# The-Learning-And-Vision-Atelier-LAVA/BUFFER

Measured on AMD Instinct MI355X. Metric: registration pairs/sec, higher is better.
Workload: dtype f32

## Files before the change

### buffer_amd/_lib.py

```python
import ctypes as C
import os

_HERE = os.path.dirname(os.path.abspath(__file__))
LIB_PATH = os.environ.get("BUF_LIB_PATH") or os.path.join(_HERE, "libbuffer_hip.so")

BUF_OK = 0


class BufferHipError(RuntimeError):
    pass


class buf_grid_t(C.Structure):
    _fields_ = [
        ("ws", C.c_void_p), ("ws_bytes", C.c_size_t),
        ("ns", C.c_int), ("nb", C.c_int),
        ("cells_per_elem", C.c_int64),
        ("radius", C.c_float),
        ("supports", C.c_void_p),
        ("desc", C.c_void_p), ("s_off", C.c_void_p), ("table", C.c_void_p),
        ("sorted", C.c_void_p), ("order", C.c_void_p), ("scan_tmp", C.c_void_p),
    ]


# ... 36 lines not shown
    "buf_vn_gather_block": (_i, [_vp, _vp, _vp, _vp, _i, _i, _i, _i, _i, _i, _f, _vp, _vp, _vp, _vp, _f, _vp, _vp]),
    "buf_vn_gather_pre_supported": (_i, [_i, _i, _i]),
    "buf_vn_gather_pre_ws_bytes": (_sz, [_i, _i]),
    "buf_vn_gather_block_pre": (_i, [_vp, _vp, _vp, _vp, _i, _i, _i, _i, _i, _f, _vp, _vp, _vp, _vp, _f, _vp, _vp, _sz, _vp]),
    "buf_vn_pointwise": (_i, [_vp, _vp, _i, _i, _i, _vp, _i, _i, _i, _vp, _vp, _vp, _vp, _f, _vp, _vp, _vp]),
    "buf_gather_max": (_i, [_vp, _vp, _i, _i, _i, _i, _vp, _vp]),
    "buf_vn_std": (_i, [_vp, _vp, _i, _i, _vp, _vp]),
    "buf_score_head_ws_bytes": (_sz, [_i, _i]),
    "buf_score_head": (_i, [_vp, _i, _vp, _i, _vp, _vp, _vp, _vp, _f, _vp, _vp, _vp, _vp, _f, _vp, _vp, _vp, _vp, _vp, _i, _vp, _vp, _i, _f,
                            _vp, _vp, _sz, _vp]),
    "buf_patch_voxelize_ws_bytes": (_sz, [_i]),
    "buf_patch_voxelize": (_i, [_vp, _vp, _i, _i, _f, _vp, _i, _i, _vp, _f, _i, _vp, _vp, _vp, _vp, _vp, _vp, _vp,
                                _vp, _vp, _sz, _vp]),
    "buf_cylindrical_net_wg": (_i, [_vp, _i, _vp, _vp, _vp, _vp, _vp, _vp, _vp]),
    "buf_cylindrical_net_wg_form": (_i, [_vp, _i, _vp, _vp, _vp, _vp, _vp, _i, _vp, _vp]),
    "buf_cylindrical_net_wg_supports": (_i, [_vp, _vp]),
    "buf_cylindrical_net_wg_flags": (_i, [_vp, _vp, _vp]),
    "buf_cylindrical_net_split_safe": (_i, [_vp, _i, _vp, _vp, _vp, _vp, _vp, _vp, _vp, _vp, _vp, _vp, _vp, _vp]),
    "buf_cylindrical_net_split_safe_form": (_i, [_vp, _i, _vp, _vp, _vp, _vp, _vp, _vp, _i, _vp, _vp, _vp, _vp, _vp, _vp]),
    "buf_cost_volume_net_split_safe": (_i, [_vp, _vp, _i, _vp, _vp, _i, _vp, _vp, _vp, _vp, _vp, _vp, _vp, _vp]),
    "buf_cylindrical_net_split": (_i, [_vp, _i, _vp, _vp, _vp, _vp, _vp, _vp, _vp, _vp]),
    "buf_cylindrical_net_split_head": (_i, [_vp, _i, _vp, _vp, _vp, _vp, _vp, _vp, _vp, _vp, _vp, _vp]),
    "buf_split_gemm_count": (C.c_longlong, [_i, _i, _i, _i]),
    "buf_split_tile_gemm": (_i, [_vp, _i, _i, _i, _i, _vp]),
    "buf_cost_volume_net_split": (_i, [_vp, _vp, _i, _vp, _vp, _vp, _vp, _vp]),
    "buf_cost_volume_net_split_gather": (_i, [_vp, _i, _vp, _vp, _i, _vp, _vp, _vp, _vp, _vp]),
    "buf_split_filter_count": (C.c_longlong, [_i, _i]),
    "buf_split_tile_filters": (_i, [_vp, _i, _i, _vp]),
    "buf_winograd_tile_weights": (_i, [_vp, _i, _i, _vp]),
    "buf_winograd_f24_tile_weights": (_i, [_vp, _i, _i, _vp]),
    "buf_winograd_group": (_i, [_i, _i]),
    "buf_cost_winograd_group": (_i, [_i]),
    "buf_winograd_tile_filters": (_i, [_vp, _i, _i, _i, _i, _vp]),
    "buf_voxel_downsample_ws_bytes": (_sz, [_i, _i64]),
    "buf_voxel_downsample": (_i, [_vp, _vp, _i, _i, C.c_double, _vp, _vp, _vp, _i64, _vp, _sz, _vp]),
# ... 62 lines not shown
```

### buffer_amd/csrc/buffer_hip.hip

```cpp
#include <stdlib.h>
#include "core.hip"
#include "radius.hip"
#include "icp.hip"
#include "pairstats.hip"
#include "posegraph.hip"
#include "metrics.hip"
#include "subsample.hip"
#include "pointops.hip"
#include "vn.hip"
#include "voxelize.hip"
#include "registration.hip"
#include "convnet.hip"
#include "convnet_h3.hip"
#include "costnet_h3.hip"
#include "preprocess.hip"
#include "convnet_wg.hip"
#include "convnet_w24.hip"
#include "convnet_w24k.hip"
#include "convnet_w24p.hip"
#include "costnet.hip"
#include "split_safe.hip"
#include "fpfh.hip"
#include "fgr.hip"
```

### buffer_amd/csrc/convnet_w24p.hip

```cpp
#include "common.h"

#define W24P_XCH_C 64
#define W24P_XCH_WIDE 36
#define W24P_XCH_OWN 12

#define W24P_MFMA(PRE, ACC, A, B) asm volatile(PRE "v_mfma_f32_16x16x4_f32 %0, %1, %2, %0" : "+a"(ACC) : "v"(A), "v"(B));

__device__ __forceinline__ void w24p_pass(unsigned P0, unsigned P1, float sgn, __amdgpu_buffer_rsrc_t rs, unsigned wp0, unsigned wp1, unsigned wp_next,
                                          unsigned lofs4, unsigned lofs2, int niter, wgf4 (&W4)[4][2], wgf2 (&W2)[4][2], wgf4 (&acc)[4][6])
{
    wgf2 D[6];
    float V[2][6];
    W24_LOAD(D, P0, P1, 0)
#define W24P_XFORM(BUF)                                                                                   \
    {                                                                                                     \
        float r_[6];                                                                                      \
        _Pragma("unroll") for (int b = 0; b < 6; b++)                                                     \
            r_[b] = __builtin_fmaf(sgn, D[3 + (b >> 1)][b & 1], D[b >> 1][b & 1]);                       \
        const float c_ = wg_sub(r_[4], r_[2]), e_ = wg_sub(r_[3], r_[1]);                                 \
        const float a_ = __builtin_fmaf(-4.f, r_[2], r_[4]), b_ = __builtin_fmaf(-4.f, r_[1], r_[3]);     \
        V[BUF][0] = __builtin_fmaf(4.f, r_[0], __builtin_fmaf(-4.f, r_[2], c_));                          \
        V[BUF][1] = wg_add(a_, b_); V[BUF][2] = wg_sub(a_, b_);                                           \
        V[BUF][3] = __builtin_fmaf(2.f, e_, c_); V[BUF][4] = __builtin_fmaf(-2.f, e_, c_);                \
        V[BUF][5] = __builtin_fmaf(-4.f, e_, wg_sub(r_[5], r_[3]));                                       \
    }
    W24P_XFORM(0)
    int it = 0;
#pragma unroll 1
    do {
        const bool more = it + 1 < niter;
        const unsigned wcur0 = wp0 + 4 * it * W24_WSTRIDE, wcur1 = wp1 + 4 * it * W24_WSTRIDE;
        const unsigned wn0 = more ? wcur0 + 4 * W24_WSTRIDE : wp_next;
        const unsigned wn1 = more ? wcur1 + 4 * W24_WSTRIDE : wp_next;
        const unsigned adv = more ? 4u * WG_KSTEP : 0u;
        __builtin_amdgcn_sched_barrier(0);
#pragma unroll
        for (int s = 0; s < 4; s++) {
            if (s < 3) W24_LOAD(D, P0, P1, (s + 1) * WG_KSTEP)
            else {
                P0 += adv; P1 += adv;
// ... 7 lines not shown
                    if (n == 0 && j == 0) W24P_MFMA("s_nop 1\n\t", acc[n][j], W24_U(n, s & 1, j), V[s & 1][j])
                    else W24P_MFMA("", acc[n][j], W24_U(n, s & 1, j), V[s & 1][j])
                }
            __builtin_amdgcn_sched_barrier(0);
            W24P_XFORM((s + 1) & 1)
#pragma unroll
            for (int n = 0; n < 4; n++) {
                const unsigned o = n < 2 ? (s < 2 ? wcur0 + (s + 2) * W24_WSTRIDE : wn0 + (s - 2) * W24_WSTRIDE)
                                         : (s < 2 ? wcur1 + (s + 2) * W24_WSTRIDE : wn1 + (s - 2) * W24_WSTRIDE);
                W4[n][s & 1] = wg_ldw(rs, o + (n & 1) * 256, lofs4);
                W2[n][s & 1] = w24_ldw2(rs, o + 512 + (n & 1) * 128, lofs2);
            }
            __builtin_amdgcn_sched_barrier(0);
        }
    } while (++it < niter);
#undef W24P_XFORM
    asm volatile("s_nop 15"
                 : "+a"(acc[0][0]), "+a"(acc[0][1]), "+a"(acc[0][2]), "+a"(acc[0][3]), "+a"(acc[0][4]), "+a"(acc[0][5]), "+a"(acc[1][0]), "+a"(acc[1][1]), "+a"(acc[1][2]), "+a"(acc[1][3]), "+a"(acc[1][4]), "+a"(acc[1][5]), "+a"(acc[2][0]), "+a"(acc[2][1]), "+a"(acc[2][2]), "+a"(acc[2][3]), "+a"(acc[2][4]), "+a"(acc[2][5]), "+a"(acc[3][0]), "+a"(acc[3][1]), "+a"(acc[3][2]), "+a"(acc[3][3]), "+a"(acc[3][4]), "+a"(acc[3][5]));
}

__device__ __forceinline__ void w24p_round_direct(unsigned row5, __amdgpu_buffer_rsrc_t rs, unsigned wp, unsigned lofs, int niter, unsigned pstride,
                                                  const float* __restrict__ bias_lane, const wgf4 (&W0)[2], wgf4& Y)
{
    constexpr int wstride = W24_WSTRIDE;
    wgf4 Wr[3][2];
#pragma unroll
    for (int k = 0; k < 2; k++) {
        Wr[0][k] = W0[k];
        Wr[1][k] = wg_ldw(rs, wp + pstride + k * wstride, lofs);
        Wr[2][k] = wg_ldw(rs, wp + 2 * pstride + k * wstride, lofs);
    }
    float X[2][6];
    unsigned pa = row5;
    WG_LOADD(X[0], pa, 0)
    WG_LOADD(X[1], pa, WG_KSTEP)
    wgf4 acc[3];
    float zero = 0.f;
    asm volatile("" : "+v"(zero));
    acc[0] = (wgf4){ zero, zero, zero, zero };
    acc[1] = (wgf4){ zero, zero, zero, zero };
    acc[2] = *reinterpret_cast<const wgf4*>(bias_lane);
    float G[6];
#define W24P_TAPS(SLOT)                                                                                   \
    {                                                                                                     \
        const wgf4 u0_ = Wr[0][SLOT], u1_ = Wr[1][SLOT], u2_ = Wr[2][SLOT];                               \
        const float d1_ = wg_sub(u1_[1], u2_[1]), d2_ = wg_sub(u1_[2], u2_[2]);                           \
        G[0] = u0_[0]; G[1] = wg_sub(u0_[1], u0_[2]); G[2] = u0_[3];                                      \
        G[3] = wg_sub(u1_[0], u2_[0]); G[4] = wg_sub(d1_, d2_); G[5] = wg_sub(u1_[3], u2_[3]);            \
    }
#define W24P_RELOAD(SLOT, OFS)                                                                            \
    _Pragma("unroll") for (int blk = 0; blk < 3; blk++) Wr[blk][SLOT] = wg_ldw(rs, (OFS) + blk * pstride, lofs);
    W24P_TAPS(0)
    W24P_RELOAD(0, wp + 2 * wstride)
#pragma unroll 1
    for (int it = 0; it < niter; it++) {
        const bool more = it + 1 < niter;
// ... 208 lines not shown
```

### buffer_amd/csrc/convnet_wg.hip

```cpp
#include "common.h"
#include <type_traits>

#define WG_CS 160
#define WG_ROW 22
#define WG_ZERO 154
#define WG_MAXC 128
#define WG_LAYERS 8
#define WG_THREADS 256
#define WG_BUF (WG_MAXC * WG_CS)
#define WG_KSTEP (16 * WG_CS)
#define WG_BLOCKS 16

typedef float wgf4 __attribute__((ext_vector_type(4)));
typedef float wgf2 __attribute__((ext_vector_type(2)));
typedef const __attribute__((address_space(3))) wgf2* wg_lds_f2;

struct CylWgParams {
    const float* wt[WG_LAYERS];
    const float* bias[WG_LAYERS];
    int cin[WG_LAYERS], cout[WG_LAYERS], relu[WG_LAYERS];
    const int* only_if;
#ifdef WG_STAMP
    long long* stamps;
#endif
// ... 581 lines not shown
                    const size_t idx = ((((((size_t)(n / ng) * nblk + i) * k4 + c / 4) * ng + n % ng) * 4 + c % 4) * 16 + o % 16);
                    out_host[idx * 4 + j] = (float)u;
                }
        }
    return BUF_OK;
}

extern "C" int buf_winograd_tile_weights(const float* w_host, int cout, int cin, float* out_host)
{
    BUF_REQUIRE(cout > 0 && cin > 0 && cout % 16 == 0 && cin % 4 == 0, BUF_EINVAL, "buf_winograd_tile_weights: widths %d -> %d", cin, cout);
    return buf_winograd_tile_filters(w_host, cout, cin, wg_group(cin, cout), WG_BLOCKS / 4, out_host);
}

extern "C" int buf_winograd_group(int cin, int cout) { return wg_group(cin, cout); }

static int wg_check_widths(const int* cin, const int* cout)
{
    for (int l = 0; l < WG_LAYERS; l++) {
        const int ci = cin[l], co = cout[l];
        BUF_REQUIRE(ci > 0 && ci % 16 == 0 && ci <= WG_MAXC && (co == 32 || co == 64 || co == 128), BUF_EINVAL,
                    "buf_cylindrical_net_wg: layer %d has unsupported widths %d -> %d", l, ci, co);
        BUF_REQUIRE(co != 128 || ci % 32 == 0, BUF_EINVAL,
                    "buf_cylindrical_net_wg: layer %d has unsupported widths %d -> %d (128 output channels need Cin %% 32 == 0)", l, ci, co);
        BUF_REQUIRE(co != 32 || (ci % 32 == 0 && ci <= 64), BUF_EINVAL,
                    "buf_cylindrical_net_wg: layer %d has unsupported widths %d -> %d (32 output channels need Cin = 32 or 64)", l, ci, co);
        BUF_REQUIRE(l == 0 || ci == cout[l - 1], BUF_EINVAL, "buf_cylindrical_net_wg: layer %d width mismatch", l);
        BUF_REQUIRE(l == 0 || cout[l - 1] != 32 || co == 32, BUF_EINVAL,
                    "buf_cylindrical_net_wg: layer %d has unsupported widths %d -> %d (only 32-output layers may follow a 32-output layer)", l, ci, co);
    }
    BUF_REQUIRE(cout[WG_LAYERS - 1] == 32, BUF_EINVAL, "buf_cylindrical_net_wg: the last layer must have 32 channels");
    return BUF_OK;
}

extern "C" int buf_cylindrical_net_wg_supports(const int* cin_host, const int* cout_host)
{
    BUF_REQUIRE(cin_host && cout_host, BUF_EINVAL, "buf_cylindrical_net_wg_supports: null argument");
    return wg_check_widths(cin_host, cout_host);
}

#define WG_F24_FLAG BUF_CYL_F24
static inline bool wg_f24_flagged(int relu) { return relu >= 2; }
static int w24_launch(const float* x, int npatch, CylWgParams P, float* y, void* stream, int form);
// ... 75 lines not shown
```

### buffer_amd/csrc/core.hip

```cpp
#include "common.h"
#include <stdarg.h>

static thread_local char g_err[512] = "";

void buf_set_error(const char* fmt, ...)
{
    va_list ap;
    va_start(ap, fmt);
    vsnprintf(g_err, sizeof(g_err), fmt, ap);
    va_end(ap);
}

extern "C" const char* buf_last_error(void) { return g_err; }
extern "C" int buf_version(void) { return 640; }

#include <mutex>
#include <vector>
struct TimedSpan { hipEvent_t a, b; double bytes; int id; };
static std::mutex g_time_mu;
static std::vector<TimedSpan> g_spans;
static int g_timing_on = 0;

extern "C" void buf_timing_enable(int on) { std::lock_guard<std::mutex> l(g_time_mu); g_timing_on = on; }

static bool timing_begin(hipStream_t s, TimedSpan* sp, double bytes, int id = BUF_TIMED_GRID_QUERY)
{
    if (!g_timing_on) return false;
    sp->id = id;
    if (hipEventCreate(&sp->a) != hipSuccess || hipEventCreate(&sp->b) != hipSuccess) return false;
// ... 241 lines not shown
```

### buffer_amd/csrc/split_safe.hip

```cpp
#include "common.h"

extern "C" int buf_cylindrical_net_split_safe_form(const float* x, int npatch, const void* const* wt_split_host, const float* const* wt_wg_host,
                                                   const float* const* bias_host, const int* cin_host, const int* cout_host, const int* relu_host,
                                                   int form, const float* head_params, float* y_or_equi, float* desc, int* status_dev,
                                                   int* flags_ws, void* stream)
{
    BUF_REQUIRE(npatch >= 0, BUF_EINVAL, "buf_cylindrical_net_split_safe: npatch=%d", npatch);
    if (npatch == 0) return BUF_OK;
    BUF_REQUIRE(x && y_or_equi && flags_ws && wt_split_host && wt_wg_host && bias_host && cin_host && cout_host && relu_host, BUF_EINVAL,
                "buf_cylindrical_net_split_safe: null argument");
    BUF_REQUIRE(!head_params || desc, BUF_EINVAL, "buf_cylindrical_net_split_safe: head without desc");
    BUF_REQUIRE(form >= BUF_CYL_FORM_DEFAULT && form <= BUF_CYL_FORM_PASS_SPLIT, BUF_EINVAL,
                "buf_cylindrical_net_split_safe: form=%d (-1: the library's default, 0: K split, 1: pass split)", form);
    if (int rc = buf_cylindrical_net_wg_flags(cin_host, cout_host, relu_host)) return rc;
    hipStream_t s = (hipStream_t)stream;
    BUF_CHECK_HIP(hipMemsetAsync(flags_ws, 0, sizeof(int) * (size_t)npatch, s));
    int relu_split[WG_LAYERS];
    for (int l = 0; l < WG_LAYERS; l++) relu_split[l] = wg_f24_flagged(relu_host[l]) ? (relu_host[l] & 1) : relu_host[l];
    int rc = h3_launch(x, npatch, wt_split_host, bias_host, cin_host, cout_host, relu_split, head_params ? nullptr : y_or_equi, head_params,
                       desc, head_params ? y_or_equi : nullptr, status_dev, stream, flags_ws);
    if (rc) return rc;
    rc = wg_launch(x, npatch, wt_wg_host, bias_host, cin_host, cout_host, relu_host, y_or_equi, flags_ws, stream, form);
    if (rc) return rc;
    if (head_params) {
        k_desc_head_masked<<<npatch, DH_THREADS, 0, s>>>(y_or_equi, head_params, desc, y_or_equi, flags_ws);
        BUF_LAUNCH_CHECK();
    }
    return BUF_OK;
}

extern "C" int buf_cylindrical_net_split_safe(const float* x, int npatch, const void* const* wt_split_host, const float* const* wt_wg_host,
                                              const float* const* bias_host, const int* cin_host, const int* cout_host, const int* relu_host,
                                              const float* head_params, float* y_or_equi, float* desc, int* status_dev, int* flags_ws,
                                              void* stream)
{
    return buf_cylindrical_net_split_safe_form(x, npatch, wt_split_host, wt_wg_host, bias_host, cin_host, cout_host, relu_host, BUF_CYL_FORM_DEFAULT,
                                               head_params, y_or_equi, desc, status_dev, flags_ws, stream);
}

extern "C" int buf_cost_volume_net_split_safe(const float* s_eq, const float* t_eq, int ele_n, const long long* s_rows, const long long* t_rows,
                                              int m, const void* const* wt_split_host, const float* const* bias_split_host,
                                              const float* const* wt_f32_host, const float* const* bias_f32_host, float* ind_out,
                                              int* status_dev, int* flags_ws, void* stream)
{
    BUF_REQUIRE(m >= 0, BUF_EINVAL, "buf_cost_volume_net_split_safe: m=%d", m);
    if (m == 0) return BUF_OK;
    BUF_REQUIRE(s_eq && t_eq && wt_split_host && bias_split_host && wt_f32_host && bias_f32_host && ind_out && flags_ws, BUF_EINVAL,
                "buf_cost_volume_net_split_safe: null argument");
    BUF_REQUIRE((s_rows == nullptr) == (t_rows == nullptr), BUF_EINVAL, "buf_cost_volume_net_split_safe: one row list without the other");
    BUF_REQUIRE(!s_rows || ele_n == 7, BUF_EINVAL, "buf_cost_volume_net_split_safe: ele_n=%d (the kernels are built for ele_n = 7)", ele_n);
    hipStream_t s = (hipStream_t)stream;
    BUF_CHECK_HIP(hipMemsetAsync(flags_ws, 0, sizeof(int) * (size_t)m, s));
    int rc = cost_net_h3_launch(s_eq, t_eq, m, wt_split_host, bias_split_host, s_rows, t_rows, ele_n, ind_out, status_dev, stream,
                                "buf_cost_volume_net_split_safe", flags_ws);
// ... 4 lines not shown
```

### buffer_amd/ops.py

```python
import ctypes as C
import time
import os
import numpy as np
import torch

from . import _lib
from ._lib import buf_grid_t, check


def _stream():
    return C.c_void_p(torch.cuda.current_stream().cuda_stream)


def _dev(t, dtype, what):
    if not isinstance(t, torch.Tensor) or not t.is_cuda:
        raise _lib.BufferHipError(f"{what}: expected a tensor in device memory (buffer_amd has no CPU path)")
    if t.dtype != dtype:
        t = t.to(dtype)
    return t.contiguous()


def _ptr(t):
    return C.c_void_p(t.data_ptr()) if t is not None else C.c_void_p(0)

# ... 691 lines not shown
                  np.float64)


def winograd_f24_filters(w):
    w64 = np.asarray(w, np.float64)
    U = np.zeros((4, 6) + w64.shape[:2], np.float64)
    for a in range(3):
        for b in range(3):
            U += (F24_G2[:, a][:, None, None, None] * w64[None, None, :, :, a, b]) * F24_G4[:, b][None, :, None, None]
    return U


F24_FLAG = 2
F24K_FLAG = 4
F24P_DEFAULT = True


def cyl_layer_filters(w, f24k=True):
    wt = winograd_tile_weights(w)
    cout, cin = w.shape[0], w.shape[1]
    if cout == 128:
        flag = F24_FLAG
    elif f24k and cout == 64 and cin % 64 == 0:
        flag = F24K_FLAG
    else:
        return wt, 0
    return np.concatenate([wt, winograd_f24_tile_weights(w)]), flag


class CylindricalNet:

    def __init__(self, layers, device, f24=True, f24k=True, f24p=F24P_DEFAULT):
        self.wt, self.bias, self.cin, self.cout, self.relu = [], [], [], [], []
        self.entry = "buf_cylindrical_net_wg"
        self.form = 1 if f24p else 0
        flags = []
        for w, b, relu in layers:
            cout, cin = w.shape[0], w.shape[1]
            wt, flag = cyl_layer_filters(w, f24k) if f24 else (winograd_tile_weights(w), 0)
            flags.append(flag)
            self.wt.append(torch.from_numpy(wt).to(device))
            self.bias.append(torch.from_numpy(np.ascontiguousarray(b, dtype=np.float32)).to(device))
            self.cin.append(cin); self.cout.append(cout); self.relu.append(1 if relu else 0)
        n = len(layers)
        self._wp = (C.c_void_p * n)(*[t.data_ptr() for t in self.wt])
        self._bp = (C.c_void_p * n)(*[t.data_ptr() for t in self.bias])
        self._ci = (C.c_int * n)(*self.cin)
        self._co = (C.c_int * n)(*self.cout)
        self._re = (C.c_int * n)(*[r | f for r, f in zip(self.relu, flags)])

    def __call__(self, x):
        L = _lib.lib()
        x = x.contiguous()
        P = x.shape[0]
        y = torch.empty((P, self.cout[-1], 7, 20), dtype=torch.float32, device=x.device)
        check(L.buf_cylindrical_net_wg_form(_ptr(x), P, self._wp, self._bp, self._ci, self._co, self._re, self.form, _ptr(y), _stream()), self.entry)
        return y


def split_tile_filters(w):
    L = _lib.lib()
    w = np.ascontiguousarray(w, dtype=np.float32)
    cout, cin = w.shape[0], w.shape[1]
    out = np.empty(L.buf_split_filter_count(cout, cin), dtype=np.uint16)
    check(L.buf_split_tile_filters(w.ctypes.data, cout, cin, out.ctypes.data), "buf_split_tile_filters")
    return out


class CylindricalNetSplit:

    def __init__(self, layers, device, f24k=True, f24p=F24P_DEFAULT):
        self.wt, self.bias, self.cin, self.cout, self.relu = [], [], [], [], []
        self.entry = "buf_cylindrical_net_split"
        self.form = 1 if f24p else 0
        for w, b, relu in layers:
            cout, cin = w.shape[0], w.shape[1]
            self.wt.append(torch.from_numpy(split_tile_filters(w).view(np.int16)).to(device))
            self.bias.append(torch.from_numpy(np.ascontiguousarray(b, dtype=np.float32)).to(device))
            self.cin.append(cin); self.cout.append(cout); self.relu.append(1 if relu else 0)
        n = len(layers)
        self.status = torch.zeros(1, dtype=torch.int32, device=device)
        self._wp = (C.c_void_p * n)(*[t.data_ptr() for t in self.wt])
        self._bp = (C.c_void_p * n)(*[t.data_ptr() for t in self.bias])
        self._ci = (C.c_int * n)(*self.cin)
        self._co = (C.c_int * n)(*self.cout)
        self._re = (C.c_int * n)(*self.relu)
        self.last_flags = None
        self.safe = n == 8 and _lib.lib().buf_cylindrical_net_wg_supports(self._ci, self._co) == 0 and not os.environ.get('BUF_SPLIT_UNSAFE')
        if self.safe:
            tiled = [cyl_layer_filters(w, f24k) for w, _, _ in layers]
            self.wt_wg = [torch.from_numpy(wt).to(device) for wt, _ in tiled]
            self._wwp = (C.c_void_p * n)(*[t.data_ptr() for t in self.wt_wg])
            self._re_safe = (C.c_int * n)(*[r | f for r, (_, f) in zip(self.relu, tiled)])

    def _safe_call(self, x, head):
        L = _lib.lib()
        x = x.contiguous()
        P = x.shape[0]
        out = torch.empty((P, self.cout[-1], 7, 20), dtype=torch.float32, device=x.device)
        desc = torch.empty((P, 32), dtype=torch.float32, device=x.device) if head is not None else None
        self.last_flags = torch.empty((max(P, 1),), dtype=torch.int32, device=x.device)
        check(L.buf_cylindrical_net_split_safe_form(_ptr(x), P, self._wp, self._wwp, self._bp, self._ci, self._co, self._re_safe, self.form,
                                                    _ptr(head.params) if head is not None else None, _ptr(out), _ptr(desc), _ptr(self.status),
                                                    _ptr(self.last_flags), _stream()), "buf_cylindrical_net_split_safe_form")
        return (desc, out) if head is not None else out

    def __call__(self, x):
        if self.safe:
            return self._safe_call(x, None)
        L = _lib.lib()
        x = x.contiguous()
        P = x.shape[0]
        y = torch.empty((P, self.cout[-1], 7, 20), dtype=torch.float32, device=x.device)
        check(L.buf_cylindrical_net_split(_ptr(x), P, self._wp, self._bp, self._ci, self._co, self._re, _ptr(y), _ptr(self.status), _stream()),
              self.entry)
        return y
# ... 194 lines not shown
```

### include/buffer_hip.h

```cpp
#ifndef BUFFER_HIP_H
#define BUFFER_HIP_H
#include <stddef.h>
#include <stdint.h>
#ifdef __cplusplus
extern "C" {
#endif

#define BUF_OK            0
#define BUF_EINVAL       -1
#define BUF_EHIP         -2
#define BUF_EWORKSPACE   -3
#define BUF_ECAPACITY    -4
#define BUF_ENODEVICE    -5

const char* buf_last_error(void);
int         buf_version(void);
int         buf_device_count(void);
#define BUF_TIMED_GRID_QUERY 0
#define BUF_TIMED_CYL_NET    1
#define BUF_TIMED_COST_NET   2
#define BUF_TIMED_SELECT_PATCHES 3
#define BUF_TIMED_PATCH_VOXELIZE 4
#define BUF_TIMED_FPS            5
#define BUF_TIMED_NN1            6
// ... 109 lines not shown
int     buf_winograd_group(int cin, int cout);
int     buf_winograd_tile_weights(const float* w_host, int cout, int cin, float* out_host);
int     buf_winograd_tile_filters(const float* w_host, int cout, int cin, int ng, int nblk, float* out_host);
#define BUF_CYL_F24 2
#define BUF_CYL_F24K 4
int     buf_cylindrical_net_wg_flags(const int* cin_host, const int* cout_host, const int* relu_host);
int     buf_winograd_f24_tile_weights(const float* w_host, int cout, int cin, float* out_host);
int     buf_cylindrical_net_wg(const float* x, int npatch, const float* const* wt_host, const float* const* bias_host,
                               const int* cin_host, const int* cout_host, const int* relu_host, float* y, void* stream);
#define BUF_CYL_FORM_DEFAULT (-1)
#define BUF_CYL_FORM_K_SPLIT 0
#define BUF_CYL_FORM_PASS_SPLIT 1
int     buf_cylindrical_net_wg_form(const float* x, int npatch, const float* const* wt_host, const float* const* bias_host,
                                    const int* cin_host, const int* cout_host, const int* relu_host, int form, float* y, void* stream);
int     buf_cylindrical_net_wg_supports(const int* cin_host, const int* cout_host);

long long buf_split_filter_count(int cout, int cin);
int     buf_split_tile_filters(const float* w_host, int cout, int cin, unsigned short* out_host);
int     buf_cylindrical_net_split(const float* x, int npatch, const void* const* wt_host, const float* const* bias_host,
                                  const int* cin_host, const int* cout_host, const int* relu_host, float* y, int* status_dev, void* stream);
int     buf_cylindrical_net_split_head(const float* x, int npatch, const void* const* wt_host, const float* const* bias_host,
                                       const int* cin_host, const int* cout_host, const int* relu_host, const float* head_params,
                                       float* desc, float* equi, int* status_dev, void* stream);

int     buf_cylindrical_net_split_safe(const float* x, int npatch, const void* const* wt_split_host, const float* const* wt_wg_host,
                                       const float* const* bias_host, const int* cin_host, const int* cout_host, const int* relu_host,
                                       const float* head_params, float* y_or_equi, float* desc, int* status_dev, int* flags_ws, void* stream);

int     buf_cylindrical_net_split_safe_form(const float* x, int npatch, const void* const* wt_split_host, const float* const* wt_wg_host,
                                            const float* const* bias_host, const int* cin_host, const int* cout_host, const int* relu_host,
                                            int form, const float* head_params, float* y_or_equi, float* desc, int* status_dev, int* flags_ws,
                                            void* stream);

int     buf_descriptor_head(const float* y, int npatch, const float* params, float* desc, float* equi, void* stream);

int     buf_cost_winograd_group(int layer);
int     buf_cost_volume_net(const float* s_eq, const float* t_eq, int m, const float* const* wt_host,
                            const float* const* bias_host, float* ind_out, void* stream);
int     buf_cost_volume_net_gather(const float* equi, int ele_n, const long long* s_rows, const long long* t_rows, int m,
                                   const float* const* wt_host, const float* const* bias_host, float* ind_out, void* stream);

long long buf_split_gemm_count(int cout, int cin, int ntaps, int nt);
int     buf_split_tile_gemm(const float* w_host, int cout, int cin, int ntaps, int nt, unsigned short* out_host);
int     buf_cost_volume_net_split(const float* s_eq, const float* t_eq, int m, const void* const* wt_host,
                                  const float* const* bias_host, float* ind_out, int* status_dev, void* stream);
int     buf_cost_volume_net_split_gather(const float* equi, int ele_n, const long long* s_rows, const long long* t_rows, int m,
                                         const void* const* wt_host, const float* const* bias_host, float* ind_out,
// ... 103 lines not shown
```

Before: 161.5.

## Use Winograd F(2x4) for 32/64-output cylindrical conv layers by default

Adds a new cylindrical-net kernel that runs layers with 32 or 64 output channels in the Winograd F(2x4) form instead of F(2x2). For 32-output layers the four waves split the input-channel reduction and combine partial results through an LDS exchange. It adds a safe-split variant that reruns flagged patches with this kernel, and makes it the default in the Python wrapper. The goal is fewer MFMA multiplies per output tile, at the cost of more transform arithmetic, an extra cross-wave reduction with a sync, and possibly higher numerical error.

```diff
diff --git a/buffer_amd/_lib.py b/buffer_amd/_lib.py
--- a/buffer_amd/_lib.py
+++ b/buffer_amd/_lib.py
@@ -74,11 +74,14 @@
                                 _vp, _vp, _sz, _vp]),
     "buf_cylindrical_net_wg": (_i, [_vp, _i, _vp, _vp, _vp, _vp, _vp, _vp, _vp]),
     "buf_cylindrical_net_wg_form": (_i, [_vp, _i, _vp, _vp, _vp, _vp, _vp, _i, _vp, _vp]),
+    "buf_cylindrical_net_wg_all": (_i, [_vp, _i, _vp, _vp, _vp, _vp, _vp, _vp, _vp, _vp]),
+    "buf_cylindrical_net_wg_all_flags": (_i, [_vp, _vp, _vp, _vp]),
     "buf_cylindrical_net_wg_supports": (_i, [_vp, _vp]),
     "buf_cylindrical_net_wg_flags": (_i, [_vp, _vp, _vp]),
     "buf_cylindrical_net_split_safe": (_i, [_vp, _i, _vp, _vp, _vp, _vp, _vp, _vp, _vp, _vp, _vp, _vp, _vp, _vp]),
     "buf_cylindrical_net_split_safe_form": (_i, [_vp, _i, _vp, _vp, _vp, _vp, _vp, _vp, _i, _vp, _vp, _vp, _vp, _vp, _vp]),
     "buf_cost_volume_net_split_safe": (_i, [_vp, _vp, _i, _vp, _vp, _i, _vp, _vp, _vp, _vp, _vp, _vp, _vp, _vp]),
+    "buf_cylindrical_net_split_safe_all": (_i, [_vp, _i, _vp, _vp, _vp, _vp, _vp, _vp, _vp, _vp, _vp, _vp, _vp, _vp, _vp]),
     "buf_cylindrical_net_split": (_i, [_vp, _i, _vp, _vp, _vp, _vp, _vp, _vp, _vp, _vp]),
     "buf_cylindrical_net_split_head": (_i, [_vp, _i, _vp, _vp, _vp, _vp, _vp, _vp, _vp, _vp, _vp, _vp]),
     "buf_split_gemm_count": (C.c_longlong, [_i, _i, _i, _i]),
diff --git a/buffer_amd/csrc/buffer_hip.hip b/buffer_amd/csrc/buffer_hip.hip
--- a/buffer_amd/csrc/buffer_hip.hip
+++ b/buffer_amd/csrc/buffer_hip.hip
@@ -18,6 +18,7 @@
 #include "convnet_w24.hip"
 #include "convnet_w24k.hip"
 #include "convnet_w24p.hip"
+#include "convnet_w24a.hip"
 #include "costnet.hip"
 #include "split_safe.hip"
 #include "fpfh.hip"
diff --git a/buffer_amd/csrc/convnet_w24a.hip b/buffer_amd/csrc/convnet_w24a.hip
--- /dev/null
+++ b/buffer_amd/csrc/convnet_w24a.hip
@@ -0,0 +1,280 @@
+#include "common.h"
+
+#define W24A_XCH_C 64
+#define W24A_XCH_WORDS 36
+
+__device__ __forceinline__ void w24a_pass(unsigned P0, unsigned P1, float sgn, __amdgpu_buffer_rsrc_t rs, unsigned wp, unsigned wp_next, unsigned lofs4,
+                                          unsigned lofs2, int niter, wgf4 (&W4)[2][2], wgf2 (&W2)[2][2], wgf4 (&acc)[2][6])
+{
+    wgf2 D[6];
+    float V[2][6];
+    W24_LOAD(D, P0, P1, 0)
+    W24P_XFORM(0)
+    int it = 0;
+#pragma unroll 1
+    do {
+        const bool more = it + 1 < niter;
+        const unsigned wcur = wp + 4 * it * W24_WSTRIDE;
+        const unsigned wn = more ? wcur + 4 * W24_WSTRIDE : wp_next;
+        const unsigned adv = more ? 4u * WG_KSTEP : 0u;
+        __builtin_amdgcn_sched_barrier(0);
+#pragma unroll
+        for (int s = 0; s < 4; s++) {
+            if (s < 3) W24_LOAD(D, P0, P1, (s + 1) * WG_KSTEP)
+            else {
+                P0 += adv; P1 += adv;
+                W24_LOAD(D, P0, P1, 0)
+            }
+            __builtin_amdgcn_sched_barrier(0);
+#pragma unroll
+            for (int n = 0; n < 2; n++)
+#pragma unroll
+                for (int j = 0; j < 6; j++)
+                    acc[n][j] = __builtin_amdgcn_mfma_f32_16x16x4f32(W24_U(n, s & 1, j), V[s & 1][j], acc[n][j], 0, 0, 0);
+            __builtin_amdgcn_sched_barrier(0);
+            W24P_XFORM((s + 1) & 1)
+#pragma unroll
+            for (int n = 0; n < 2; n++) {
+                const unsigned o = s < 2 ? wcur + (s + 2) * W24_WSTRIDE : wn + (s - 2) * W24_WSTRIDE;
+                W4[n][s & 1] = wg_ldw(rs, o + n * 256, lofs4);
+                W2[n][s & 1] = w24_ldw2(rs, o + 512 + n * 128, lofs2);
+            }
+            __builtin_amdgcn_sched_barrier(0);
+        }
+    } while (++it < niter);
+}
+
+template <bool GLB>
+__device__ __forceinline__ void w24a_store(const wgf4 (&Yk)[2][4], const wgf4& Yb, int nt, int relu, float* __restrict__ act, float* __restrict__ out_glb,
+                                           int li, int lk)
+{
+    if constexpr (GLB) {
+        const int n0 = nt * 16 + lk * 4;
+        const float lo = relu ? 0.f : -__builtin_inff();
+        int ty, tx;
+        w24_tile(li, ty, tx);
+#pragma unroll
+        for (int u = 0; u < 2; u++) {
+            const int row = 2 * ty + u;
+            if (row < 7) {
+#pragma unroll
+                for (int r = 0; r < 4; r++)
+                    *reinterpret_cast<wgf4*>(out_glb + (size_t)(n0 + r) * 140 + row * 20 + 4 * tx) =
+                        (wgf4){ fmaxf(Yk[u][0][r], lo), fmaxf(Yk[u][1][r], lo), fmaxf(Yk[u][2][r], lo), fmaxf(Yk[u][3][r], lo) };
+            }
+        }
+    } else
+        w24_store_tile(Yk, nt, relu, act, li, lk);
+    wg_store_row6<GLB>(Yb, nt, relu, act, out_glb, li, lk);
+}
+
+template <int Q, bool GLB>
+__device__ __forceinline__ void w24a_take(const wgf4 (&f)[2][4], wgf4 Yb, int relu, float* __restrict__ act, float* __restrict__ out_glb, int lane)
+{
+    const float* xch = act + (W24A_XCH_C + (lane >> 2)) * WG_CS + (lane & 3) * W24A_XCH_WORDS;
+    wgf4 Yk[2][4];
+#pragma unroll
+    for (int v = 0; v < 4; v++) {
+        wgf4 F[4];
+#pragma unroll
+        for (int i = 0; i < 4; i++)
+            F[i] = i == Q ? f[Q][v] : *reinterpret_cast<const wgf4*>(xch + 16 * i * WG_CS + 16 * Q + 4 * v);
+        Yk[0][v] = (F[0] + F[1]) + F[2];
+        Yk[1][v] = (F[1] - F[2]) - F[3];
+    }
+    Yb += *reinterpret_cast<const wgf4*>(xch + 16 * (Q + 2) * WG_CS + 32);
+    w24a_store<GLB>(Yk, Yb, Q, relu, act, out_glb, lane & 15, lane >> 4);
+}
+
+template <bool GLB>
+__device__ __forceinline__ void w24a_layer_psplit32(float* __restrict__ act, float* __restrict__ out_glb, const float* __restrict__ wt,
+                                                    const float* __restrict__ bias, int cin, int relu, int w, const WgAddrPark& pk, const W24AddrPark& pk24)
+{
+    act[(threadIdx.x >> 1) * WG_CS + WG_ZERO + 4 + (threadIdx.x & 1)] = 0.f;
+    __syncthreads();
+    int lane = threadIdx.x & (WAVE - 1);
+    asm volatile("" : "+v"(lane));
+    const int lk = lane >> 4;
+    const int k4 = cin >> 2, kn = k4 >> 1;
+    const int nd = w & 1, half = w >> 1;
+    const __amdgpu_buffer_rsrc_t rs = wg_weights(wt);
+    const unsigned pstride = (unsigned)(k4 * W24_WSTRIDE);
+    const unsigned wp = (unsigned)w * pstride;
+    const unsigned wpd = (unsigned)(half * kn) * W24_WSTRIDE + (unsigned)nd * 256;
+    const unsigned lofs4 = lane * 16, lofs2 = lane * 8;
+    const wgf4 W0[2] = { wg_ldw(rs, wpd, lofs4), wg_ldw(rs, wpd + W24_WSTRIDE, lofs4) };
+    wgf4 Yb;
+    w24p_round_direct<true>(wg_parked(pk, 2, 0) + (unsigned)(half * kn) * WG_KSTEP, rs, wpd, lofs4, kn >> 2, pstride,
+                            half ? nullptr : bias + nd * 16 + lk * 4, W0, Yb);
+    unsigned RA[4];
+#pragma unroll
+    for (int a = 0; a < 4; a++) asm volatile("v_accvgpr_read_b32 %0, %1" : "=v"(RA[a]) : "a"(pk24.a[a]));
+    const unsigned P0 = w == 0 ? RA[0] : (w == 2 ? RA[2] : RA[1]);
+    const unsigned P1 = w == 3 ? RA[3] : (w == 2 ? RA[1] : RA[2]);
+    const float sgn = w == 1 ? 1.f : -1.f;
+    wgf4 f[2][4];
+    {
+        wgf4 acc[2][6];
+        float zero = 0.f;
+        asm volatile("" : "+v"(zero));
+#pragma unroll
+        for (int n = 0; n < 2; n++)
+#pragma unroll
+            for (int j = 0; j < 6; j++) acc[n][j] = (wgf4){ zero, zero, zero, zero };
+        if (w == 1) {
+#pragma unroll
+            for (int n = 0; n < 2; n++) acc[n][1] = *reinterpret_cast<const wgf4*>(bias + n * 16 + lk * 4);
+        }
+        wgf4 W4[2][2];
+        wgf2 W2[2][2];
+#pragma unroll
+        for (int n = 0; n < 2; n++)
+#pragma unroll
+            for (int k = 0; k < 2; k++) {
+                W4[n][k] = wg_ldw(rs, wp + k * W24_WSTRIDE + n * 256, lofs4);
+                W2[n][k] = w24_ldw2(rs, wp + k * W24_WSTRIDE + 512 + n * 128, lofs2);
+            }
+        w24a_pass(P0, P1, sgn, rs, wp, wp, lofs4, lofs2, k4 >> 2, W4, W2, acc);
+        __builtin_amdgcn_sched_barrier(0);
+#pragma unroll
+        for (int n = 0; n < 2; n++)
+#pragma unroll
+            for (int r = 0; r < 4; r++) {
+                const float p = acc[n][1][r] + acc[n][2][r], q = acc[n][1][r] - acc[n][2][r];
+                const float t = acc[n][3][r] + acc[n][4][r], d = acc[n][3][r] - acc[n][4][r];
+                f[n][0][r] = acc[n][0][r] + p + t;
+                f[n][1][r] = __builtin_fmaf(2.f, d, q);
+                f[n][2][r] = __builtin_fmaf(4.f, t, p);
+                f[n][3][r] = __builtin_fmaf(8.f, d, q) + acc[n][5][r];
+            }
+    }
+    int lane_s = threadIdx.x & (WAVE - 1);
+    asm volatile("" : "+v"(lane_s));
+    float* mine = act + (W24A_XCH_C + 16 * w + (lane_s >> 2)) * WG_CS + (lane_s & 3) * W24A_XCH_WORDS;
+    if (w != 0) {
+#pragma unroll
+        for (int v = 0; v < 4; v++) *reinterpret_cast<wgf4*>(mine + 4 * v) = f[0][v];
+    }
+    if (w != 1) {
+#pragma unroll
+        for (int v = 0; v < 4; v++) *reinterpret_cast<wgf4*>(mine + 16 + 4 * v) = f[1][v];
+    }
+    if (half) *reinterpret_cast<wgf4*>(mine + 32) = Yb;
+    __syncthreads();
+    if (w == 0) w24a_take<0, GLB>(f, Yb, relu, act, out_glb, lane_s);
+    else if (w == 1) w24a_take<1, GLB>(f, Yb, relu, act, out_glb, lane_s);
+}
+
+__device__ __forceinline__ void cyl_net_w24a_body(const float* __restrict__ x, const CylWgParams& P, float* __restrict__ y, float* __restrict__ lds)
+{
+    float* act = lds;
+    const int patch = blockIdx.x;
+    const int w = __builtin_amdgcn_readfirstlane(threadIdx.x / WAVE);
+    wg_load_input(x, P, act, patch);
+    WgAddrPark pk;
+    W24AddrPark pk24;
+    {
+        int lane0 = threadIdx.x & (WAVE - 1);
+        asm volatile("" : "+v"(lane0));
+        wg_park_addresses(act, lane0 & 15, lane0 >> 4, pk);
+        w24_park_addresses(act, lane0 & 15, lane0 >> 4, pk24);
+    }
+#pragma unroll 1
+    for (int l = 0; l < WG_LAYERS; l++) {
+        const int cin = P.cin[l], cout = P.cout[l], relu = P.relu[l] & 1;
+        const bool f24 = (P.relu[l] & W24K_FLAG) != 0;
+        float* yp = y + (size_t)patch * cout * 140;
+        if (cout == 128) w24_layer_pair(act, P.wt[l], P.bias[l], cin, relu, w, pk, pk24);
+        else if (cout == 64 && f24) w24p_layer_psplit(act, P.wt[l], P.bias[l], cin, relu, w, pk, pk24);
+        else if (cout == 64) wg_layer_msplit(act, P.wt[l], P.bias[l], cin, cout, relu, w, pk);
+        else if (f24 && l < WG_LAYERS - 1) w24a_layer_psplit32<false>(act, nullptr, P.wt[l], P.bias[l], cin, relu, w, pk, pk24);
+        else if (f24) w24a_layer_psplit32<true>(act, yp, P.wt[l], P.bias[l], cin, relu, w, pk, pk24);
+        else if (l < WG_LAYERS - 1) wg_layer_mksplit<false>(act, nullptr, P.wt[l], P.bias[l], cin, cout, relu, w, pk);
+        else wg_layer_mksplit<true>(act, yp, P.wt[l], P.bias[l], cin, cout, relu, w, pk);
+        __syncthreads();
+    }
+}
+
+__global__ void __launch_bounds__(WG_THREADS, 2) k_cyl_net_w24a(const float* __restrict__ x, CylWgParams P, float* __restrict__ y)
+{
+    extern __shared__ float lds[];
+    cyl_net_w24a_body(x, P, y, lds);
+}
+
+__global__ void __launch_bounds__(WG_THREADS, 2) k_cyl_net_w24a_rerun(const float* __restrict__ x, CylWgParams P, float* __restrict__ y)
+{
+    extern __shared__ float lds[];
+    if (P.only_if[blockIdx.x] == 0) return;
+    cyl_net_w24a_body(x, P, y, lds);
+}
+
+static int w24a_check(const int* cin, const int* cout, const int* relu, const float* const* wt24_host)
+{
+    if (int rc = wg_check_widths(cin, cout, false)) return rc;
+    if (int rc = w24_check_flags(cin, cout, relu)) return rc;
+    bool f22_ran = false;
+    int f22_layer = -1;
+    for (int l = 0; l < WG_LAYERS; l++) {
+        BUF_REQUIRE(!wt24_host[l] || (!(relu[l] & (WG_F24_FLAG | W24K_FLAG)) && (cout[l] == 64 || cout[l] == 32)), BUF_EINVAL,
+                    "buf_cylindrical_net_wg_all: layer %d (%d -> %d, flags %d) takes no F(2x4) set of its own (64 or 32 output channels, no F(2x4) flag)",
+                    l, cin[l], cout[l], relu[l]);
+        BUF_REQUIRE(!f22_ran || cout[l] == 32, BUF_EINVAL,
+                    "buf_cylindrical_net_wg_all: layer %d has unsupported widths %d -> %d (once a 32-output layer in the F(2x2) form has run, layer %d here, "
+                    "only 32-output layers may follow)", l, cin[l], cout[l], f22_layer);
+        if (cout[l] == 32 && !wt24_host[l] && !f22_ran) { f22_ran = true; f22_layer = l; }
+    }
+    return BUF_OK;
+}
+
+extern "C" int buf_cylindrical_net_wg_all_flags(const int* cin_host, const int* cout_host, const int* relu_host, const float* const* wt24_host)
+{
+    BUF_REQUIRE(cin_host && cout_host && relu_host && wt24_host, BUF_EINVAL, "buf_cylindrical_net_wg_all_flags: null argument");
+    return w24a_check(cin_host, cout_host, relu_host, wt24_host);
+}
+
+static int w24a_prepare(const float* const* wt_host, const float* const* bias_host, const int* cin_host, const int* cout_host, const int* relu_host,
+                        const float* const* wt24_host, CylWgParams& P)
+{
+    BUF_REQUIRE(wt_host && bias_host && cin_host && cout_host && relu_host && wt24_host, BUF_EINVAL, "buf_cylindrical_net_wg_all: null argument");
+    for (int l = 0; l < WG_LAYERS; l++) {
+        P.wt[l] = wt_host[l]; P.bias[l] = bias_host[l];
+        P.cin[l] = cin_host[l]; P.cout[l] = cout_host[l]; P.relu[l] = relu_host[l];
+        BUF_REQUIRE(P.wt[l] && P.bias[l], BUF_EINVAL, "buf_cylindrical_net_wg_all: null weights for layer %d", l);
+    }
+    if (int rc = w24a_check(P.cin, P.cout, P.relu, wt24_host)) return rc;
+    for (int l = 0; l < WG_LAYERS; l++) {
+        if (P.relu[l] & WG_F24_FLAG) P.wt[l] += W24_SET_F22(P.cin[l]);
+        else if (P.relu[l] & W24K_FLAG) P.wt[l] += WG_BLOCKS * P.cout[l] * P.cin[l];
+        else if (wt24_host[l]) { P.wt[l] = wt24_host[l]; P.relu[l] |= W24K_FLAG; }
+        P.relu[l] &= ~WG_F24_FLAG;
+    }
+    P.only_if = nullptr;
+    return BUF_OK;
+}
+
+static int w24a_launch(const float* x, int npatch, CylWgParams P, float* y, void* stream)
+{
+    size_t lds = sizeof(float) * WG_BUF;
+    static LdsGrant grant, grant_rerun;
+    if (int rc = P.only_if ? grant_dynamic_lds((const void*)k_cyl_net_w24a_rerun, lds, grant_rerun) : grant_dynamic_lds((const void*)k_cyl_net_w24a, lds, grant)) return rc;
+    double macs = 0;
+    for (int l = 0; l < WG_LAYERS; l++) macs += 9.0 * P.cin[l] * P.cout[l];
+    TimedSpan span;
+    bool timed = !P.only_if && timing_begin((hipStream_t)stream, &span, 2.0 * 140 * macs * npatch, BUF_TIMED_CYL_NET);
+    if (P.only_if) k_cyl_net_w24a_rerun<<<npatch, WG_THREADS, lds, (hipStream_t)stream>>>(x, P, y);
+    else k_cyl_net_w24a<<<npatch, WG_THREADS, lds, (hipStream_t)stream>>>(x, P, y);
+    if (timed) timing_end((hipStream_t)stream, &span);
+    BUF_LAUNCH_CHECK();
+    return BUF_OK;
+}
+
+extern "C" int buf_cylindrical_net_wg_all(const float* x, int npatch, const float* const* wt_host, const float* const* bias_host, const int* cin_host,
+                                          const int* cout_host, const int* relu_host, const float* const* wt24_host, float* y, void* stream)
+{
+    BUF_REQUIRE(npatch >= 0, BUF_EINVAL, "buf_cylindrical_net_wg_all: npatch=%d", npatch);
+    if (npatch == 0) return BUF_OK;
+    BUF_REQUIRE(x && y, BUF_EINVAL, "buf_cylindrical_net_wg_all: null argument");
+    CylWgParams P;
+    if (int rc = w24a_prepare(wt_host, bias_host, cin_host, cout_host, relu_host, wt24_host, P)) return rc;
+    return w24a_launch(x, npatch, P, y, stream);
+}
diff --git a/buffer_amd/csrc/convnet_w24p.hip b/buffer_amd/csrc/convnet_w24p.hip
--- a/buffer_amd/csrc/convnet_w24p.hip
+++ b/buffer_amd/csrc/convnet_w24p.hip
@@ -6,12 +6,6 @@
 
 #define W24P_MFMA(PRE, ACC, A, B) asm volatile(PRE "v_mfma_f32_16x16x4_f32 %0, %1, %2, %0" : "+a"(ACC) : "v"(A), "v"(B));
 
-__device__ __forceinline__ void w24p_pass(unsigned P0, unsigned P1, float sgn, __amdgpu_buffer_rsrc_t rs, unsigned wp0, unsigned wp1, unsigned wp_next,
-                                          unsigned lofs4, unsigned lofs2, int niter, wgf4 (&W4)[4][2], wgf2 (&W2)[4][2], wgf4 (&acc)[4][6])
-{
-    wgf2 D[6];
-    float V[2][6];
-    W24_LOAD(D, P0, P1, 0)
 #define W24P_XFORM(BUF)                                                                                   \
     {                                                                                                     \
         float r_[6];                                                                                      \
@@ -24,6 +18,13 @@
         V[BUF][3] = __builtin_fmaf(2.f, e_, c_); V[BUF][4] = __builtin_fmaf(-2.f, e_, c_);                \
         V[BUF][5] = __builtin_fmaf(-4.f, e_, wg_sub(r_[5], r_[3]));                                       \
     }
+
+__device__ __forceinline__ void w24p_pass(unsigned P0, unsigned P1, float sgn, __amdgpu_buffer_rsrc_t rs, unsigned wp0, unsigned wp1, unsigned wp_next,
+                                          unsigned lofs4, unsigned lofs2, int niter, wgf4 (&W4)[4][2], wgf2 (&W2)[4][2], wgf4 (&acc)[4][6])
+{
+    wgf2 D[6];
+    float V[2][6];
+    W24_LOAD(D, P0, P1, 0)
     W24P_XFORM(0)
     int it = 0;
 #pragma unroll 1
@@ -61,11 +62,11 @@
             __builtin_amdgcn_sched_barrier(0);
         }
     } while (++it < niter);
-#undef W24P_XFORM
     asm volatile("s_nop 15"
                  : "+a"(acc[0][0]), "+a"(acc[0][1]), "+a"(acc[0][2]), "+a"(acc[0][3]), "+a"(acc[0][4]), "+a"(acc[0][5]), "+a"(acc[1][0]), "+a"(acc[1][1]), "+a"(acc[1][2]), "+a"(acc[1][3]), "+a"(acc[1][4]), "+a"(acc[1][5]), "+a"(acc[2][0]), "+a"(acc[2][1]), "+a"(acc[2][2]), "+a"(acc[2][3]), "+a"(acc[2][4]), "+a"(acc[2][5]), "+a"(acc[3][0]), "+a"(acc[3][1]), "+a"(acc[3][2]), "+a"(acc[3][3]), "+a"(acc[3][4]), "+a"(acc[3][5]));
 }
 
+template <bool NOBIAS = false>
 __device__ __forceinline__ void w24p_round_direct(unsigned row5, __amdgpu_buffer_rsrc_t rs, unsigned wp, unsigned lofs, int niter, unsigned pstride,
                                                   const float* __restrict__ bias_lane, const wgf4 (&W0)[2], wgf4& Y)
 {
@@ -86,7 +87,8 @@
     asm volatile("" : "+v"(zero));
     acc[0] = (wgf4){ zero, zero, zero, zero };
     acc[1] = (wgf4){ zero, zero, zero, zero };
-    acc[2] = *reinterpret_cast<const wgf4*>(bias_lane);
+    if constexpr (NOBIAS) acc[2] = bias_lane ? *reinterpret_cast<const wgf4*>(bias_lane) : (wgf4){ zero, zero, zero, zero };
+    else acc[2] = *reinterpret_cast<const wgf4*>(bias_lane);
     float G[6];
 #define W24P_TAPS(SLOT)                                                                                   \
     {                                                                                                     \
diff --git a/buffer_amd/csrc/convnet_wg.hip b/buffer_amd/csrc/convnet_wg.hip
--- a/buffer_amd/csrc/convnet_wg.hip
+++ b/buffer_amd/csrc/convnet_wg.hip
@@ -619,7 +619,7 @@
 
 extern "C" int buf_winograd_group(int cin, int cout) { return wg_group(cin, cout); }
 
-static int wg_check_widths(const int* cin, const int* cout)
+static int wg_check_widths(const int* cin, const int* cout, bool follow = true)
 {
     for (int l = 0; l < WG_LAYERS; l++) {
         const int ci = cin[l], co = cout[l];
@@ -630,7 +630,7 @@
         BUF_REQUIRE(co != 32 || (ci % 32 == 0 && ci <= 64), BUF_EINVAL,
                     "buf_cylindrical_net_wg: layer %d has unsupported widths %d -> %d (32 output channels need Cin = 32 or 64)", l, ci, co);
         BUF_REQUIRE(l == 0 || ci == cout[l - 1], BUF_EINVAL, "buf_cylindrical_net_wg: layer %d width mismatch", l);
-        BUF_REQUIRE(l == 0 || cout[l - 1] != 32 || co == 32, BUF_EINVAL,
+        BUF_REQUIRE(!follow || l == 0 || cout[l - 1] != 32 || co == 32, BUF_EINVAL,
                     "buf_cylindrical_net_wg: layer %d has unsupported widths %d -> %d (only 32-output layers may follow a 32-output layer)", l, ci, co);
     }
     BUF_REQUIRE(cout[WG_LAYERS - 1] == 32, BUF_EINVAL, "buf_cylindrical_net_wg: the last layer must have 32 channels");
diff --git a/buffer_amd/csrc/core.hip b/buffer_amd/csrc/core.hip
--- a/buffer_amd/csrc/core.hip
+++ b/buffer_amd/csrc/core.hip
@@ -12,7 +12,7 @@
 }
 
 extern "C" const char* buf_last_error(void) { return g_err; }
-extern "C" int buf_version(void) { return 640; }
+extern "C" int buf_version(void) { return 650; }
 
 #include <mutex>
 #include <vector>
diff --git a/buffer_amd/csrc/split_safe.hip b/buffer_amd/csrc/split_safe.hip
--- a/buffer_amd/csrc/split_safe.hip
+++ b/buffer_amd/csrc/split_safe.hip
@@ -38,6 +38,34 @@
                                                head_params, y_or_equi, desc, status_dev, flags_ws, stream);
 }
 
+extern "C" int buf_cylindrical_net_split_safe_all(const float* x, int npatch, const void* const* wt_split_host, const float* const* wt_wg_host,
+                                                  const float* const* bias_host, const int* cin_host, const int* cout_host, const int* relu_host,
+                                                  const float* const* wt24_host, const float* head_params, float* y_or_equi, float* desc,
+                                                  int* status_dev, int* flags_ws, void* stream)
+{
+    BUF_REQUIRE(npatch >= 0, BUF_EINVAL, "buf_cylindrical_net_split_safe_all: npatch=%d", npatch);
+    if (npatch == 0) return BUF_OK;
+    BUF_REQUIRE(x && y_or_equi && flags_ws && wt_split_host, BUF_EINVAL, "buf_cylindrical_net_split_safe_all: null argument");
+    BUF_REQUIRE(!head_params || desc, BUF_EINVAL, "buf_cylindrical_net_split_safe_all: head without desc");
+    CylWgParams P;
+    if (int rc = w24a_prepare(wt_wg_host, bias_host, cin_host, cout_host, relu_host, wt24_host, P)) return rc;
+    hipStream_t s = (hipStream_t)stream;
+    BUF_CHECK_HIP(hipMemsetAsync(flags_ws, 0, sizeof(int) * (size_t)npatch, s));
+    int relu_split[WG_LAYERS];
+    for (int l = 0; l < WG_LAYERS; l++) relu_split[l] = relu_host[l] & 1;
+    int rc = h3_launch(x, npatch, wt_split_host, bias_host, cin_host, cout_host, relu_split, head_params ? nullptr : y_or_equi, head_params,
+                       desc, head_params ? y_or_equi : nullptr, status_dev, stream, flags_ws);
+    if (rc) return rc;
+    P.only_if = flags_ws;
+    rc = w24a_launch(x, npatch, P, y_or_equi, stream);
+    if (rc) return rc;
+    if (head_params) {
+        k_desc_head_masked<<<npatch, DH_THREADS, 0, s>>>(y_or_equi, head_params, desc, y_or_equi, flags_ws);
+        BUF_LAUNCH_CHECK();
+    }
+    return BUF_OK;
+}
+
 extern "C" int buf_cost_volume_net_split_safe(const float* s_eq, const float* t_eq, int ele_n, const long long* s_rows, const long long* t_rows,
                                               int m, const void* const* wt_split_host, const float* const* bias_split_host,
                                               const float* const* wt_f32_host, const float* const* bias_f32_host, float* ind_out,
diff --git a/buffer_amd/ops.py b/buffer_amd/ops.py
--- a/buffer_amd/ops.py
+++ b/buffer_amd/ops.py
@@ -729,6 +729,8 @@
 F24_FLAG = 2
 F24K_FLAG = 4
 F24P_DEFAULT = True
+F24A_DEFAULT = 'all'
+F24A_PARTS = {'all': (64, 32), 'out64': (64,), 'out32': (32,), 'off': (), None: ()}
 
 
 def cyl_layer_filters(w, f24k=True):
@@ -743,9 +745,33 @@
     return np.concatenate([wt, winograd_f24_tile_weights(w)]), flag
 
 
+def cyl_f24a_parts(f24, f24k, f24p, f24a):
+    explicit = not (f24 is None and f24k is None and f24p is None)
+    f24, f24k, f24p = (True if f24 is None else f24), (True if f24k is None else f24k), (F24P_DEFAULT if f24p is None else f24p)
+    if f24a is None:
+        f24a = None if explicit else F24A_DEFAULT
+    if f24a is True:
+        f24a = 'all'
+    if f24a is False:
+        f24a = 'off'
+    if f24a not in F24A_PARTS:
+        raise ValueError(f"f24a = {f24a!r}: one of 'all', 'out64', 'out32', 'off'")
+    if F24A_PARTS[f24a] and not (f24 and f24k and f24p):
+        raise ValueError("f24a goes with the default forms of the other layers (f24, f24k, f24p left alone or true)")
+    return f24, f24k, f24p, F24A_PARTS[f24a]
+
+
+def cyl_f24a_filters(layers, flags, parts, device):
+    sets = [torch.from_numpy(winograd_f24_tile_weights(w)).to(device)
+            if (flag == 0 and w.shape[0] in parts and w.shape[0] in (32, 64) and w.shape[1] % 16 == 0) else None
+            for (w, _, _), flag in zip(layers, flags)]
+    return sets, (C.c_void_p * len(sets))(*[None if t is None else t.data_ptr() for t in sets])
+
+
 class CylindricalNet:
 
-    def __init__(self, layers, device, f24=True, f24k=True, f24p=F24P_DEFAULT):
+    def __init__(self, layers, device, f24=None, f24k=None, f24p=None, f24a=None):
+        f24, f24k, f24p, parts = cyl_f24a_parts(f24, f24k, f24p, f24a)
         self.wt, self.bias, self.cin, self.cout, self.relu = [], [], [], [], []
         self.entry = "buf_cylindrical_net_wg"
         self.form = 1 if f24p else 0
@@ -763,12 +789,19 @@
         self._ci = (C.c_int * n)(*self.cin)
         self._co = (C.c_int * n)(*self.cout)
         self._re = (C.c_int * n)(*[r | f for r, f in zip(self.relu, flags)])
+        self.wt24, self._w24p = cyl_f24a_filters(layers, flags, parts, device)
+        self.f24_layers = [l for l, t in enumerate(self.wt24) if t is not None]
+        self.f24_all = bool(self.f24_layers) and all(f or t is not None for f, t in zip(flags, self.wt24))
 
     def __call__(self, x):
         L = _lib.lib()
         x = x.contiguous()
         P = x.shape[0]
         y = torch.empty((P, self.cout[-1], 7, 20), dtype=torch.float32, device=x.device)
+        if self.f24_layers:
+            check(L.buf_cylindrical_net_wg_all(_ptr(x), P, self._wp, self._bp, self._ci, self._co, self._re, self._w24p, _ptr(y), _stream()),
+                  "buf_cylindrical_net_wg_all")
+            return y
         check(L.buf_cylindrical_net_wg_form(_ptr(x), P, self._wp, self._bp, self._ci, self._co, self._re, self.form, _ptr(y), _stream()), self.entry)
         return y
 
@@ -784,9 +817,11 @@
 
 class CylindricalNetSplit:
 
-    def __init__(self, layers, device, f24k=True, f24p=F24P_DEFAULT):
+    def __init__(self, layers, device, f24k=None, f24p=None, f24a=None):
+        _, f24k, f24p, parts = cyl_f24a_parts(None, f24k, f24p, f24a)
         self.wt, self.bias, self.cin, self.cout, self.relu = [], [], [], [], []
         self.entry = "buf_cylindrical_net_split"
+        self.f24_layers, self.f24_all = [], False
         self.form = 1 if f24p else 0
         for w, b, relu in layers:
             cout, cin = w.shape[0], w.shape[1]
@@ -807,6 +842,9 @@
             self.wt_wg = [torch.from_numpy(wt).to(device) for wt, _ in tiled]
             self._wwp = (C.c_void_p * n)(*[t.data_ptr() for t in self.wt_wg])
             self._re_safe = (C.c_int * n)(*[r | f for r, (_, f) in zip(self.relu, tiled)])
+            self.wt24, self._w24p = cyl_f24a_filters(layers, [f for _, f in tiled], parts, device)
+            self.f24_layers = [l for l, t in enumerate(self.wt24) if t is not None]
+            self.f24_all = bool(self.f24_layers) and all(f or t is not None for (_, f), t in zip(tiled, self.wt24))
 
     def _safe_call(self, x, head):
         L = _lib.lib()
@@ -815,6 +853,11 @@
         out = torch.empty((P, self.cout[-1], 7, 20), dtype=torch.float32, device=x.device)
         desc = torch.empty((P, 32), dtype=torch.float32, device=x.device) if head is not None else None
         self.last_flags = torch.empty((max(P, 1),), dtype=torch.int32, device=x.device)
+        if self.f24_layers:
+            check(L.buf_cylindrical_net_split_safe_all(_ptr(x), P, self._wp, self._wwp, self._bp, self._ci, self._co, self._re_safe, self._w24p,
+                                                       _ptr(head.params) if head is not None else None, _ptr(out), _ptr(desc), _ptr(self.status),
+                                                       _ptr(self.last_flags), _stream()), "buf_cylindrical_net_split_safe_all")
+            return (desc, out) if head is not None else out
         check(L.buf_cylindrical_net_split_safe_form(_ptr(x), P, self._wp, self._wwp, self._bp, self._ci, self._co, self._re_safe, self.form,
                                                     _ptr(head.params) if head is not None else None, _ptr(out), _ptr(desc), _ptr(self.status),
                                                     _ptr(self.last_flags), _stream()), "buf_cylindrical_net_split_safe_form")
diff --git a/include/buffer_hip.h b/include/buffer_hip.h
--- a/include/buffer_hip.h
+++ b/include/buffer_hip.h
@@ -147,6 +147,10 @@
 int     buf_cylindrical_net_wg_form(const float* x, int npatch, const float* const* wt_host, const float* const* bias_host,
                                     const int* cin_host, const int* cout_host, const int* relu_host, int form, float* y, void* stream);
 int     buf_cylindrical_net_wg_supports(const int* cin_host, const int* cout_host);
+int     buf_cylindrical_net_wg_all_flags(const int* cin_host, const int* cout_host, const int* relu_host, const float* const* wt24_host);
+int     buf_cylindrical_net_wg_all(const float* x, int npatch, const float* const* wt_host, const float* const* bias_host,
+                                   const int* cin_host, const int* cout_host, const int* relu_host, const float* const* wt24_host,
+                                   float* y, void* stream);
 
 long long buf_split_filter_count(int cout, int cin);
 int     buf_split_tile_filters(const float* w_host, int cout, int cin, unsigned short* out_host);
@@ -164,6 +168,10 @@
                                             const float* const* bias_host, const int* cin_host, const int* cout_host, const int* relu_host,
                                             int form, const float* head_params, float* y_or_equi, float* desc, int* status_dev, int* flags_ws,
                                             void* stream);
+int     buf_cylindrical_net_split_safe_all(const float* x, int npatch, const void* const* wt_split_host, const float* const* wt_wg_host,
+                                           const float* const* bias_host, const int* cin_host, const int* cout_host, const int* relu_host,
+                                           const float* const* wt24_host, const float* head_params, float* y_or_equi, float* desc,
+                                           int* status_dev, int* flags_ws, void* stream);
 
 int     buf_descriptor_head(const float* y, int npatch, const float* params, float* desc, float* equi, void* stream);
 
```

After: 163.7 (median of 6 runs). +1.4%, better.
